# Chen001117/mappo

Hardware: AMD Instinct MI355X
Metric: agent-steps/sec (collect+GAE+PPO), MPE simple_spread 3-agent (higher is better)
Workload: dtype f32; 1 GPU; BASELINE configs[1]: MPE simple_spread shape, 3 agents, obs 18 / share_obs 54 / Discrete(5), n_rollout_threads=1024 in total (strong scaling: 1024 on rank 0 of 1), episode_length=25, MLP policy (mappo), ppo_epoch=10, num_mini_batch=1, lr 7e-4, env=synthetic; n_rollout_threads_global=1024, n_rollout_threads_rank0=1024, episode_length=25, num_agents=3, ppo_epoch=10, num_mini_batch=1, parallelism=dp1, rccl_ranks=0, exact_minibatch_order=False, hip_graph=True

## Files before the change

mappo_amd/csrc/insert_core.h:

```cpp
#pragma once
#include "common.h"

struct InsertArgs {
  const float *obs;  int64_t obs_sn, obs_sm;
  const float *rew;  int64_t rew_sn, rew_sm;
  const uint8_t *done; int64_t done_sn, done_sm;
  float *obs_dst, *share_dst, *rew_dst, *mask_dst;
  int N, M, D, centralized;
};

__device__ __forceinline__ void insert_mpe_body(const InsertArgs &p, int bid, int nb) {
  const int S = p.centralized ? p.M * p.D : p.D;
  const int64_t total = (int64_t)p.N * p.M * S;
  for (int64_t e = (int64_t)bid * blockDim.x + threadIdx.x; e < total; e += (int64_t)nb * blockDim.x) {
    const int64_t nm = e / S;
    const int j = (int)(e - nm * S);
    const int n = (int)(nm / p.M), m = (int)(nm - (int64_t)n * p.M);
    const int ms = p.centralized ? j / p.D : m, d = p.centralized ? j - ms * p.D : j;
    const float v = p.obs[n * p.obs_sn + ms * p.obs_sm + d];
    p.share_dst[e] = v;
    if (!p.centralized || ms == m) p.obs_dst[nm * p.D + d] = v;
    if (j == 0) {
      p.rew_dst[nm] = p.rew[n * p.rew_sn + m * p.rew_sm];
      p.mask_dst[nm] = p.done[n * p.done_sn + m * p.done_sm] ? 0.f : 1.f;
    }
  }
}

template <int U>
__device__ __forceinline__ void insert_mpe_episode_body(const InsertArgs &p, int64_t obs_st, int64_t rew_st, int64_t done_st, int T,
                                                        int bid, int nb) {
  const int S = p.centralized ? p.M * p.D : p.D;
  const int64_t R = (int64_t)p.N * p.M, RS = R * S, total = (int64_t)T * RS, nthr = (int64_t)nb * blockDim.x;
  for (int64_t e0 = (int64_t)bid * blockDim.x + threadIdx.x; e0 < total; e0 += U * nthr) {
    float v[U], rw[U];
    uint8_t dn[U];
    int64_t tn[U];
    int dd[U], jj[U];
#pragma unroll
    for (int u = 0; u < U; ++u) {
      const int64_t e = e0 + u * nthr;
      jj[u] = -1;
      if (e < total) {
        const int64_t t = e / RS, rem = e - t * RS, nm = rem / S;
        const int j = (int)(rem - nm * S);
        const int n = (int)(nm / p.M), m = (int)(nm - (int64_t)n * p.M);
        const int ms = p.centralized ? j / p.D : m, d = p.centralized ? j - ms * p.D : j;
        v[u] = p.obs[t * obs_st + n * p.obs_sn + ms * p.obs_sm + d];
        tn[u] = t * R + nm;
        dd[u] = (!p.centralized || ms == m) ? d : -1;
        jj[u] = j;
        if (j == 0) {
          rw[u] = p.rew[t * rew_st + n * p.rew_sn + m * p.rew_sm];
          dn[u] = p.done[t * done_st + n * p.done_sn + m * p.done_sm];
        }
      }
    }
    __builtin_amdgcn_sched_barrier(0);
    __builtin_amdgcn_s_waitcnt(0);
    __builtin_amdgcn_sched_barrier(0);
#pragma unroll
    for (int u = 0; u < U; ++u) {
      if (jj[u] < 0) continue;
      p.share_dst[e0 + u * nthr] = v[u];
      if (dd[u] >= 0) p.obs_dst[tn[u] * p.D + dd[u]] = v[u];
      if (jj[u] == 0) {
        p.rew_dst[tn[u]] = rw[u];
        p.mask_dst[tn[u]] = dn[u] != 0 ? 0.f : 1.f;
      }
    }
  }
}

struct SmacInsert {
  const float *obs, *share, *avail;
  const float *rew; int64_t rew_sn, rew_sm;
  const uint8_t *done; int64_t done_sn, done_sm;
  const uint8_t *bad;
  const float *h_a, *h_c;
  float *obs_dst, *share_dst, *avail_dst, *rew_dst, *mask_dst, *bad_dst, *active_dst, *ha_dst, *hc_dst;
  int N, M, D, S, A, H;
};
__device__ __forceinline__ bool env_done(const SmacInsert &p, int n) {
  bool all = true;
  for (int m = 0; m < p.M; ++m) all = all && p.done[n * p.done_sn + m * p.done_sm] != 0;
  return all;
}
__device__ __forceinline__ void insert_smac_body(const SmacInsert &p, int bid, int nb) {
  const int64_t tid = (int64_t)bid * blockDim.x + threadIdx.x, nthr = (int64_t)nb * blockDim.x;
  const int64_t R = (int64_t)p.N * p.M;
  for (int64_t e = tid; e < R * p.D; e += nthr) p.obs_dst[e] = p.obs[e];
  for (int64_t e = tid; e < R * p.S; e += nthr) p.share_dst[e] = p.share[e];
  if (p.avail)
    for (int64_t e = tid; e < R * p.A; e += nthr) p.avail_dst[e] = p.avail[e];
  for (int64_t e = tid; e < R; e += nthr) {
    const int n = (int)(e / p.M), m = (int)(e - (int64_t)n * p.M);
    const bool de = env_done(p, n), d = p.done[n * p.done_sn + m * p.done_sm] != 0;
    p.rew_dst[e] = p.rew[n * p.rew_sn + m * p.rew_sm];
    p.mask_dst[e] = de ? 0.f : 1.f;
    p.active_dst[e] = de ? 1.f : (d ? 0.f : 1.f);
    p.bad_dst[e] = (p.bad && p.bad[e]) ? 0.f : 1.f;
  }
  if (p.h_a) {
    const int h4 = p.H >> 2;
    for (int64_t e = tid; e < R * h4; e += nthr) {
      const int n = (int)((e / h4) / p.M);
      const float keep = env_done(p, n) ? 0.f : 1.f;
      float4 a = reinterpret_cast<const float4 *>(p.h_a)[e], c = reinterpret_cast<const float4 *>(p.h_c)[e];
      a.x *= keep; a.y *= keep; a.z *= keep; a.w *= keep;
      c.x *= keep; c.y *= keep; c.z *= keep; c.w *= keep;
      reinterpret_cast<float4 *>(p.ha_dst)[e] = a;
      reinterpret_cast<float4 *>(p.hc_dst)[e] = c;
    }
  }
}
```

mappo_amd/csrc/mlp_fwd16.h:

```cpp
#pragma once

#include "mlp_trunk16r.h"

template <bool RELU>
__device__ __forceinline__ void act_ln16(f32x4 (&acc)[4], const float *sG, const float *sBt, int q) {
  float s = 0.f;
#pragma unroll
  for (int b = 0; b < 4; ++b)
#pragma unroll
    for (int r = 0; r < 4; ++r) { acc[b][r] = act_fwd<RELU>(acc[b][r]); s += acc[b][r]; }
  const float mean = quad_sum16(s) * (1.f / HID);
  float v = 0.f;
#pragma unroll
  for (int b = 0; b < 4; ++b)
#pragma unroll
    for (int r = 0; r < 4; ++r) { const float c = acc[b][r] - mean; v += c * c; }
  const float rstd = 1.0f / sqrtf(quad_sum16(v) * (1.f / HID) + LN_EPS);
#pragma unroll
  for (int b = 0; b < 4; ++b) {
    const float4 g = *reinterpret_cast<const float4 *>(sG + 16 * b + 4 * q), t = *reinterpret_cast<const float4 *>(sBt + 16 * b + 4 * q);
    acc[b][0] = (acc[b][0] - mean) * rstd * g.x + t.x;
    acc[b][1] = (acc[b][1] - mean) * rstd * g.y + t.y;
    acc[b][2] = (acc[b][2] - mean) * rstd * g.z + t.z;
    acc[b][3] = (acc[b][3] - mean) * rstd * g.w + t.w;
// ... 126 lines not shown
  } else {
    f32x4 z[NBH > 0 ? NBH : 1];
#pragma unroll
    for (int bo = 0; bo < NBH; ++bo) {
      z[bo] = hd.bhv[bo];
      if (bo == 0 || A > 16) {
#pragma unroll
        for (int b = 0; b < 4; ++b)
#pragma unroll
          for (int r = 0; r < 4; ++r) z[bo] = mfma16(hd.wh[bo][b][r], h[b][r], z[bo]);
      }
    }
    if constexpr (DRAIN) { __builtin_amdgcn_sched_barrier(0); __builtin_amdgcn_s_waitcnt(0); __builtin_amdgcn_sched_barrier(0); }
    if constexpr (MODE == 0) {
      if (A == 1) { if (ok && q == 0) out[i] = z[0][0]; }
      else if (ok) {
#pragma unroll
        for (int r = 0; r < 4; ++r) { const int a = 4 * q + r; if (a < A) out[i * A + a] = z[0][r]; }
      }
    } else {
#pragma unroll
      for (int bo = 0; bo < NBH; ++bo)
#pragma unroll
        for (int r = 0; r < 4; ++r) { const int a = 16 * bo + 4 * q + r; if (a < A) tZ[j * TP + a] = z[bo][r]; }
      wave_lds_sync();
      if (ok && q == 0) {
        const uint64_t ctr = ctr_base + (ctr_dev ? *ctr_dev : 0ull);
        float action, lp;
        categorical_act_lane(tZ + j * TP, A, p.avail ? p.avail + i * A : nullptr, p.deterministic != 0, p.seed, ctr, (uint64_t)i, action, lp);
        actions[i] = action;
        logp[i] = lp;
      }
      wave_lds_sync();
    }
  }
}

template <bool RELU, int LN, int MODE>
__device__ __forceinline__ void forward16r_body(const FwdArgs &p, float *lds, const int bid, const int nb) {
  const int n_waves = blockDim.x / WAVE;
  const NetOff &o = p.off;
  const int lane = threadIdx.x & (WAVE - 1), wave = __builtin_amdgcn_readfirstlane((int)(threadIdx.x / WAVE)), j = lane & 15, q = lane >> 4;
  const int D = p.desc.in_dim, A = p.desc.out_dim;
  const int64_t n_tiles = (p.B + 15) / 16;
  float *tZ = lds + wave * 16 * TP;
  int64_t tile = (int64_t)bid * n_waves + wave;
  if (tile >= n_tiles) return;
  const float *P = p.params;
  auto load_x = [&](int64_t tl, f32x4 (&xv)[4]) {
    const int64_t i = tl * 16 + j;
    const int64_t row = i < p.B ? (p.rows ? (int64_t)p.rows[i] : i) : 0;
    const int64_t off = p.x_M ? (row / p.x_M) * p.x_sn + (row % p.x_M) * p.x_sm : row * D;
#pragma unroll
    for (int b = 0; b < 4; ++b)
#pragma unroll
      for (int r = 0; r < 4; ++r) xv[b][r] = p.x[off + min(16 * b + 4 * q + r, D - 1)];
  };
  f32x4 xn[4];
  load_x(tile, xn);
  Trunk16R<LN> tw;
  trunk16r_load<LN>(tw, P, o, p.desc, j, q);
  Head16R<MODE> hd;
  head16r_load<MODE>(hd, P, o, A, j, q);
  for (; tile < n_tiles; tile += (int64_t)nb * n_waves) {
    const int64_t i = tile * 16 + j;
    const bool ok = i < p.B;
    f32x4 x[4];
#pragma unroll
    for (int b = 0; b < 4; ++b) x[b] = xn[b];
    if (tile + (int64_t)nb * n_waves < n_tiles) load_x(tile + (int64_t)nb * n_waves, xn);
    tile16r_step<RELU, LN, MODE>(p, tw, hd, x, p.out, p.actions, p.logp, p.counter, p.counter_dev, tZ, i, ok, j, q);
  }
}

struct EpisodeSrc {
  const float *x0;
  int64_t x0_sn, x0_sm;
  const float *xp;
  int64_t xp_st, xp_sn, xp_sm;
};

template <bool RELU, int LN, int MODE>
__device__ __forceinline__ void episode16r_body(const FwdArgs &p, const EpisodeSrc &s, const int M, const int n_steps, const int n_last,
                                                float *last_out, float *lds, const int bid, const int nb) {
  const int n_waves = blockDim.x / WAVE;
  const int lane = threadIdx.x & (WAVE - 1), wave = __builtin_amdgcn_readfirstlane((int)(threadIdx.x / WAVE)), j = lane & 15, q = lane >> 4;
  const int D = p.desc.in_dim, A = p.desc.out_dim;
  const int64_t n_tiles = (p.B + 15) / 16;
  float *tZ = lds + wave * 16 * TP;
  const int64_t tile0 = (int64_t)bid * n_waves + wave, tstride = (int64_t)nb * n_waves;
  if (tile0 >= n_tiles) return;
  const int n_my = (int)((n_tiles - tile0 + tstride - 1) / tstride);
  const int n_items = n_steps * n_my;
  auto load_x = [&](int it, f32x4 (&xv)[4]) {
    const int t = it / n_my, k = it - t * n_my;
    const int64_t i = (tile0 + k * tstride) * 16 + j;
    const int64_t row = i < p.B ? i : 0;
    const float *base = t == 0 ? s.x0 : s.xp + (int64_t)(t - 1) * s.xp_st;
    const int64_t sn = t == 0 ? s.x0_sn : s.xp_sn, sm = t == 0 ? s.x0_sm : s.xp_sm;
    const int64_t off = (row / M) * sn + (row % M) * sm;
#pragma unroll
    for (int b = 0; b < 4; ++b)
#pragma unroll
      for (int r = 0; r < 4; ++r) xv[b][r] = base[off + min(16 * b + 4 * q + r, D - 1)];
  };
  f32x4 xn[4];
  load_x(0, xn);
  Trunk16R<LN> tw;
  trunk16r_load<LN>(tw, p.params, p.off, p.desc, j, q);
  Head16R<MODE> hd;
  head16r_load<MODE>(hd, p.params, p.off, A, j, q);
  const uint64_t ctr0 = p.counter + (MODE == 1 && p.counter_dev ? *p.counter_dev : 0ull);
  __builtin_amdgcn_sched_barrier(0);
  __builtin_amdgcn_s_waitcnt(0);
  __builtin_amdgcn_sched_barrier(0);
  for (int it = 0; it < n_items; ++it) {
    const int t = it / n_my, k = it - t * n_my;
    const int64_t i = (tile0 + k * tstride) * 16 + j;
    const bool ok = i < p.B;
    f32x4 x[4];
#pragma unroll
    for (int b = 0; b < 4; ++b) x[b] = xn[b];
    if (it + 1 < n_items) load_x(it + 1, xn);
    const int64_t so = (int64_t)t * p.B;
    float *out = MODE == 0 ? (t == n_last ? last_out : p.out + so) : nullptr;
    tile16r_step<RELU, LN, MODE, true>(p, tw, hd, x, out, MODE == 1 ? p.actions + so : nullptr, MODE == 1 ? p.logp + so : nullptr,
                                       ctr0 + (uint64_t)t, nullptr, tZ, i, ok, j, q);
  }
}

template <bool RELU, int LN, int MODE>
__device__ __forceinline__ void forward16_body(const FwdArgs &p, float *lds, const int bid, const int nb) {
  const int n_waves = blockDim.x / WAVE;
  const NetOff &o = p.off;
  const LdsMap &m = p.map;
  const int lane = threadIdx.x & (WAVE - 1), wave = __builtin_amdgcn_readfirstlane((int)(threadIdx.x / WAVE)), j = lane & 15, q = lane >> 4;
  const int D = p.desc.in_dim, Dp = (D + 1) & ~1, A = p.desc.out_dim;
  const int NG = (D + 3) >> 2;
  const int64_t n_tiles = (p.B + 15) / 16;
  const bool fnorm = p.desc.use_feature_norm != 0;
  const float inv_D = 1.0f / (float)D;
  float *tZ = lds + m.tiles + wave * m.wave_stride;
  bool staged = false;
  for (int64_t tile = (int64_t)bid * n_waves + wave; tile < n_tiles || !staged; tile += (int64_t)nb * n_waves) {
    const int64_t i = tile * 16 + j;
    const bool ok = tile < n_tiles && i < p.B;
    const int64_t row = ok ? (p.rows ? (int64_t)p.rows[i] : i) : 0;
    const int64_t off = p.x_M ? (row / p.x_M) * p.x_sn + (row % p.x_M) * p.x_sm : row * D;
    float xin[16];
#pragma unroll
    for (int g = 0; g < 16; ++g) xin[g] = p.x[off + min(4 * g + q, D - 1)];
    if (!staged) {
      stage_all_weights_1shot<LN>(lds, m, p.params, o, p.desc);
      __syncthreads();
      staged = true;
      if (tile >= n_tiles) break;
    }
#pragma unroll
    for (int g = 0; g < 16; ++g) xin[g] = (ok && 4 * g + q < D) ? xin[g] : 0.f;
    if (fnorm) {
      float s = 0.f;
#pragma unroll
      for (int g = 0; g < 16; ++g) s += xin[g];
      const float mean = quad_sum16(s) * inv_D;
      float v = 0.f;
#pragma unroll
      for (int g = 0; g < 16; ++g) { const float c = xin[g] - mean; v += c * c; }
      const int n_empty = 16 - max(0, min(16, (D - q + 3) >> 2));
      v -= (float)n_empty * mean * mean;
      const float rstd = 1.0f / sqrtf(fmaxf(quad_sum16(v), 0.f) * inv_D + LN_EPS);
#pragma unroll
      for (int g = 0; g < 16; ++g) xin[g] = (xin[g] - mean) * rstd * lds[m.fn_w + 4 * g + q] + lds[m.fn_b + 4 * g + q];
    }
    f32x4 h[4];
#pragma unroll
    for (int b = 0; b < 4; ++b) {
      const float4 bv = *reinterpret_cast<const float4 *>(lds + m.b1 + 16 * b + 4 * q);
      h[b][0] = bv.x; h[b][1] = bv.y; h[b][2] = bv.z; h[b][3] = bv.w;
    }
#pragma unroll
    for (int c = 0; c < 4; ++c) {
      if (4 * c < NG) {
#pragma unroll
        for (int gg = 0; gg < 4; ++gg) {
          const int g = 4 * c + gg;
          const float *rowp = lds + m.w1 + min(4 * g + q, Dp - 1) * WP + j;
#pragma unroll
          for (int b = 0; b < 4; ++b) h[b] = mfma16(rowp[16 * b], xin[g], h[b]);
        }
      }
    }
    forward16_tail<RELU, LN, MODE>(p, lds, m, h, i, ok, j, q, tZ);
  }
}
```

mappo_amd/csrc/mlp_impl.h:

```cpp
#include "mlp_core.h"
#include <stdlib.h>

#ifdef MLP_TU_MAIN
extern "C" int64_t mappo_net_param_count(const mappo_net_desc *desc) {
  if (!desc) return -1;
  return net_offsets(*desc).total;
}
#endif

struct LdsMap {
  int w1, w2[MAPPO_MAX_LAYER_N], wh;
  int fn_w, fn_b, b1, ln1_w, ln1_b, b2[MAPPO_MAX_LAYER_N], ln2_w[MAPPO_MAX_LAYER_N], ln2_b[MAPPO_MAX_LAYER_N], bh;
  int scratch;
  int tiles, x_rows, wave_stride, total;
  int fn_size;
};


__host__ __device__ inline LdsMap lds_map(const mappo_net_desc &d, int n_waves) {
  LdsMap m;
  int p = 0;
  const bool xw = d.in_dim > MAXD;
  const int Dp = xw ? MAXD : ((d.in_dim + 1) & ~1);
  m.fn_size = xw ? ((d.in_dim + 63) / 64) * 64 : MAXD;
// ... 522 lines not shown
    const int64_t base = tile * TS;
    int n_valid;
    TileStats<LN> st;
    if (!XWIDE) {
      n_valid = pf.n_valid;
      commit_rows(tX, tH + ((4 - ((m.x_rows * TP) & 3)) & 3), pf, D, magic, lane, p.desc.use_feature_norm != 0);
      wave_lds_sync();
      prefetch_rows(pf, p.x, p.rows, (tile + tile_stride) * TS, p.B, D, lane, p.x_sn, p.x_sm, p.x_M);
      tile_forward<RELU, LN>(lds, m, tX, tH, D, l31, half, st);
    } else {
      n_valid = (int)max((int64_t)0, min((int64_t)TS, p.B - base));
      const bool ok = l31 < n_valid;
      const int64_t row = ok ? (p.rows ? (int64_t)p.rows[base + l31] : base + l31) : 0;
      const float *xr = p.x + row * D;
      float mean0, rstd0;
      wide_row_stats(xr, D, ok, half, p.desc.use_feature_norm != 0, mean0, rstd0);
      tile_forward_wide<RELU, LN>(lds, m, p.params + o.w1, xr, ok, mean0, rstd0, tX, tH, D, l31, half, st);
    }
    if (MODE == 2) {
      const float *tL = tH + LN * HID * TP, *sG = lds + ln_w_of<LN>(m, LN), *sBt = lds + ln_b_of<LN>(m, LN);
      if (l31 < n_valid) {
#pragma unroll
        for (int t = 0; t < 2; ++t)
#pragma unroll
          for (int r = 0; r < 16; ++r) {
            const int f = 32 * t + ROWMAP(r, half);
            p.out[(int64_t)f * p.B + base + l31] = tL[f * TP + l31] * sG[f] + sBt[f];
          }
      }
      wave_lds_sync();
      continue;
    }
    const f32x16 z = head_forward(lds, m, tH + LN * HID * TP, lds + ln_w_of<LN>(m, LN), lds + ln_b_of<LN>(m, LN), l31, half);
    head_to_tile(tZ, z, A, l31, half);
    wave_lds_sync();
    if (MODE == 0) {
      for (int e = lane; e < n_valid * A; e += WAVE) {
        const int s = e / A, a = e - s * A;
        p.out[base * A + e] = tZ[s * TP + a];
      }
    } else {
      if (lane < n_valid) {
        const int64_t i = base + lane;
        const uint64_t ctr = p.counter + (p.counter_dev ? *p.counter_dev : 0ull);
        float action, logp;
        categorical_act_lane(tZ + lane * TP, A, p.avail ? p.avail + i * A : nullptr, p.deterministic != 0, p.seed, ctr, (uint64_t)i,
                             action, logp);
        p.actions[i] = action;
        p.logp[i] = logp;
      }
    }
    wave_lds_sync();
  }
}

template <bool RELU, int LN, int MODE, int XW>
__global__ __launch_bounds__(256, 1) void mlp_forward_kernel(FwdArgs p) {
  extern __shared__ __align__(16) float lds[];
  forward_body<RELU, LN, MODE, XW>(p, lds, blockIdx.x, gridDim.x);
}

#include "insert_core.h"
struct StepArgs {
  FwdArgs a, c;
  InsertArgs ins;
  int nA, nC, nI;
};
#include "mlp_fwd16.h"
template <bool RELU, int LN>
__global__ __launch_bounds__(256, 1) void rollout_step_kernel(StepArgs s) {
  extern __shared__ __align__(16) float lds[];
  const int bid = blockIdx.x;
  if (bid < s.nA) forward16r_body<RELU, LN, 1>(s.a, lds, bid, s.nA);
  else if (bid < s.nA + s.nC) forward16r_body<RELU, LN, 0>(s.c, lds, bid - s.nA, s.nC);
  else insert_mpe_body(s.ins, bid - s.nA - s.nC, s.nI);
}

struct EpisodeArgs {
  FwdArgs a, c;
  EpisodeSrc sa, sc;
  float *next_values;
  InsertArgs ins;
  int64_t ins_obs_st, ins_rew_st, ins_done_st;
  int T, M, nA, nC, nI;
};
template <bool RELU, int LN>
__global__ __launch_bounds__(256, 1) void rollout_episode_kernel(EpisodeArgs e) {
  extern __shared__ __align__(16) float lds[];
  const int bid = blockIdx.x;
  if (bid < e.nA) episode16r_body<RELU, LN, 1>(e.a, e.sa, e.M, e.T, -1, nullptr, lds, bid, e.nA);
  else if (bid < e.nA + e.nC) episode16r_body<RELU, LN, 0>(e.c, e.sc, e.M, e.T + 1, e.T, e.next_values, lds, bid - e.nA, e.nC);
  else insert_mpe_episode_body<8>(e.ins, e.ins_obs_st, e.ins_rew_st, e.ins_done_st, e.T, bid - e.nA - e.nC, e.nI);
}

template <bool RELU, int LN>
__global__ __launch_bounds__(256, 1) void features16_kernel(FwdArgs a) {
  extern __shared__ __align__(16) float lds[];
  forward16r_body<RELU, LN, 2>(a, lds, blockIdx.x, gridDim.x);
}
template <bool RELU, int LN>
__global__ __launch_bounds__(256, 1) void features16_dual_kernel(FwdArgs a, FwdArgs c, int nA) {
  extern __shared__ __align__(16) float lds[];
  if ((int)blockIdx.x < nA) forward16r_body<RELU, LN, 2>(a, lds, blockIdx.x, nA);
  else forward16r_body<RELU, LN, 2>(c, lds, blockIdx.x - nA, gridDim.x - nA);
}

#ifdef MLP_STAMPS
#define N_STAMPS 24
static unsigned long long *g_stamp_host = nullptr;
#define STAMP_DECL unsigned long long st_acc_[N_STAMPS] = {}; unsigned long long st_prev_ = __builtin_readcyclecounter();
#define STAMP(i)                                                          \
  do {                                                                    \
    __builtin_amdgcn_sched_barrier(0);                                    \
    const unsigned long long now_ = __builtin_readcyclecounter();         \
    st_acc_[i] += now_ - st_prev_;                                        \
    st_prev_ = now_;                                                      \
    __builtin_amdgcn_sched_barrier(0);                                    \
  } while (0)
#define STAMP_FLUSH()                                                                     \
  do {                                                                                    \
    if (p.stamps && threadIdx.x == 0)                                                     \
      for (int i_ = 0; i_ < N_STAMPS; ++i_) p.stamps[blockIdx.x * N_STAMPS + i_] = st_acc_[i_]; \
  } while (0)
#ifdef MLP_TU_MAIN
extern "C" int mappo_debug_set_stamps(unsigned long long *buf) { g_stamp_host = buf; return 0; }
#endif
#else
#define STAMP_DECL
#define STAMP(i) do { } while (0)
#define STAMP_FLUSH() do { } while (0)
#endif

struct UpdArgs {
  const float *params, *x;
  const int32_t *rows;
  float *slabs;
  int64_t slab_stride, slab_col0;
  mappo_net_desc desc;
  NetOff off;
  LdsMap map;
  int64_t B;
  int n_blocks;
  int n_regions;
  int p_red;
  int red_base;
  float *wide_ws;
  const float *dHT;
  int seq_nc;
  const float *dout;
  const float *avail, *actions, *old_logp, *adv, *active, *v_old, *returns, *vn_state;
  const double *mb_moments;
  double *partials;
  mappo_ppo_cfg cfg;
  unsigned long long *stamps;
};

__device__ __forceinline__ float tile_row_sum(const float *tile, int lane) {
  float s0 = 0.f, s1 = 0.f;
#pragma unroll 4
  for (int j = 0; j < TS; j += 2) { s0 += tile[lane * TP + j]; s1 += tile[lane * TP + j + 1]; }
  return s0 + s1;
}

__device__ __forceinline__ void regs_to_tile(float *tile, const f32x16 (&v)[2], int l31, int half) {
#pragma unroll
  for (int t = 0; t < 2; ++t)
#pragma unroll
    for (int r = 0; r < 16; ++r) tile[(32 * t + ROWMAP(r, half)) * TP + l31] = v[t][r];
}

template <bool RELU, bool AFFINE>
__device__ __forceinline__ void ln_act_backward(f32x16 (&dH)[2], float *tile, float mean, float rstd, uint32_t pos,
                                                const float *sG, float &gG, float &gB, int lane, int l31, int half) {
  f32x16 xh[2];
#pragma unroll
// ... 1067 lines not shown
    FwdArgs a = {}, c = {};
    a.params = actor_params; a.x = obs; a.avail = avail; a.actions = actions; a.logp = logp; a.desc = *actor_desc; a.B = B;
    a.deterministic = deterministic; a.seed = seed; a.counter = counter; a.counter_dev = counter_dev;
    a.off = net_offsets(a.desc); a.map = lds_map(a.desc, 8);
    c.params = critic_params; c.x = share_obs; c.out = values; c.desc = *critic_desc; c.B = B; c.off = net_offsets(c.desc); c.map = lds_map(c.desc, 8);
    Wide16Args wa, wc;
    size_t lba, lbc;
    dim3 ga, gc, ba, bc;
    bool sa, sc;
    if (int rcp = wide_forward_prepare(a, wa, lba, ga, ba, sa, "rollout_step")) return rcp;
    if (int rcp = wide_forward_prepare(c, wc, lbc, gc, bc, sc, "rollout_step")) return rcp;
    wa.x_M = M; wa.x_sn = obs_stride_n; wa.x_sm = obs_stride_m;
    wc.x_M = M; wc.x_sn = share_stride_n; wc.x_sm = share_stride_m;
    const int64_t n_groups = ((B + 15) / 16 + 7) / 8;
    const int nb = (int)(n_groups < NUM_CU / 2 ? n_groups : NUM_CU / 2);
    const int nA = actions ? nb : 0;
    const dim3 grid((unsigned)(nA + nb));
    const size_t lb = lba > lbc ? lba : lbc;
    if (full_step) {
      const size_t lw = sizeof(float) * ((size_t)HID * actor_desc->in_dim + HID);
      const size_t lf = lw > lb ? lw : lb;
      MAPPO_REQUIRE(lf <= 159 * 1024, "rollout_step: needs %zu B of LDS", lf);
      InsertArgs ins = {};
      if (fuse_ins) {
        wa.copy_dst = obs_dst; wc.copy_dst = share_dst;
        ins.rew = rewards; ins.rew_sn = rew_stride_n; ins.rew_sm = rew_stride_m; ins.done = dones; ins.done_sn = done_stride_n;
        ins.done_sm = done_stride_m; ins.rew_dst = rew_dst; ins.mask_dst = mask_dst; ins.N = (int)(B / M); ins.M = M;
      }
      const int rcf = actor_desc->use_relu
          ? wide16_launch_rollout_full_r<true>(actor_desc->layer_N, grid, lf, as_stream(stream), wa, a, wc, c, nA, fuse_ins ? &ins : nullptr)
          : wide16_launch_rollout_full_r<false>(actor_desc->layer_N, grid, lf, as_stream(stream), wa, a, wc, c, nA, fuse_ins ? &ins : nullptr);
      if (rcf) return rcf;
      MAPPO_CHECK_LAUNCH("rollout_step");
      return MAPPO_OK;
    }
    const int rcw = actor_desc->use_relu ? wide16_launch_rollout_step_r<true>(actor_desc->layer_N, grid, lb, as_stream(stream), wa, a, wc, c, nA)
                                         : wide16_launch_rollout_step_r<false>(actor_desc->layer_N, grid, lb, as_stream(stream), wa, a, wc, c, nA);
    if (rcw) return rcw;
    MAPPO_CHECK_LAUNCH("rollout_step");
    return MAPPO_OK;
  }
  const int64_t n_tiles = (B + 15) / 16;
  const int want = n_tiles >= 4 ? 4 : (n_tiles >= 2 ? 2 : 1);
  int nw = fit_waves(*actor_desc, want);
  const int nwc = fit_waves(*critic_desc, want);
  nw = nw < nwc ? nw : nwc;
  StepArgs s = {};
  s.a.params = actor_params; s.a.x = obs; s.a.avail = avail; s.a.actions = actions; s.a.logp = logp; s.a.desc = *actor_desc; s.a.B = B;
  s.a.deterministic = deterministic; s.a.seed = seed; s.a.counter = counter; s.a.counter_dev = counter_dev;
  s.a.x_sn = obs_stride_n; s.a.x_sm = obs_stride_m; s.a.x_M = M;
  s.a.off = net_offsets(s.a.desc); s.a.map = lds_map(s.a.desc, nw);
  s.c.params = critic_params; s.c.x = share_obs; s.c.out = values; s.c.desc = *critic_desc; s.c.B = B;
  s.c.x_sn = share_stride_n; s.c.x_sm = share_stride_m; s.c.x_M = M;
  s.c.off = net_offsets(s.c.desc); s.c.map = lds_map(s.c.desc, nw);
  const int totA = s.a.map.total, totC = s.c.map.total;
  const size_t lds_bytes = (size_t)(totA > totC ? totA : totC) * sizeof(float);
  MAPPO_REQUIRE(lds_bytes <= LDS_DYN_MAX, "rollout_step: needs %zu B of LDS", lds_bytes);
  int64_t nb = (n_tiles + nw - 1) / nw;
  if (nb > NUM_CU / 2) nb = NUM_CU / 2;
  s.nA = actions ? (int)nb : 0; s.nC = (int)nb; s.nI = 0;
  if (obs_dst) {
    InsertArgs &i = s.ins;
    i.obs = obs; i.obs_sn = obs_stride_n; i.obs_sm = obs_stride_m; i.rew = rewards; i.rew_sn = rew_stride_n; i.rew_sm = rew_stride_m;
    i.done = dones; i.done_sn = done_stride_n; i.done_sm = done_stride_m; i.obs_dst = obs_dst; i.share_dst = share_dst;
    i.rew_dst = rew_dst; i.mask_dst = mask_dst; i.N = (int)(B / M); i.M = M; i.D = actor_desc->in_dim; i.centralized = centralized;
    const int64_t total = B * (centralized ? (int64_t)M * i.D : i.D);
    int64_t ni = (total + 2047) / 2048;
    s.nI = (int)(ni > NUM_CU ? NUM_CU : ni);
  }
  dim3 grid((unsigned)(s.nA + s.nC + s.nI)), block(WAVE * nw);
  const bool relu = actor_desc->use_relu != 0;
  int rc;
  switch (actor_desc->layer_N) {
    case 0: rc = relu ? step_launch<true, 0>(grid, block, lds_bytes, as_stream(stream), s) : step_launch<false, 0>(grid, block, lds_bytes, as_stream(stream), s); break;
    case 1: rc = relu ? step_launch<true, 1>(grid, block, lds_bytes, as_stream(stream), s) : step_launch<false, 1>(grid, block, lds_bytes, as_stream(stream), s); break;
    default: rc = relu ? step_launch<true, 2>(grid, block, lds_bytes, as_stream(stream), s) : step_launch<false, 2>(grid, block, lds_bytes, as_stream(stream), s); break;
  }
  if (rc) return rc;
  MAPPO_CHECK_LAUNCH("rollout_step");
  return MAPPO_OK;
}

#define EPISODE_WAVES 1
template <bool R, int L>
static int episode_launch(dim3 grid, dim3 block, size_t lds_bytes, hipStream_t st, const EpisodeArgs &a) {
  hipLaunchKernelGGL((rollout_episode_kernel<R, L>), grid, block, lds_bytes, st, a);
  return MAPPO_OK;
}

extern "C" int mappo_rollout_episode(const float *actor_params, const mappo_net_desc *actor_desc, const float *critic_params,
                                     const mappo_net_desc *critic_desc, int32_t T, int32_t N, int32_t M, const float *env_obs,
                                     int64_t obs_stride_t, int64_t obs_stride_n, int64_t obs_stride_m, const float *rewards,
                                     int64_t rew_stride_t, int64_t rew_stride_n, int64_t rew_stride_m, const uint8_t *dones,
                                     int64_t done_stride_t, int64_t done_stride_n, int64_t done_stride_m, int32_t deterministic,
                                     uint64_t seed, uint64_t counter, const uint64_t *counter_dev, float *obs_buf, float *share_buf,
                                     float *rew_buf, float *mask_buf, float *actions, float *logp, float *values, float *next_values,
                                     int32_t centralized, mappo_stream_t stream) {
  if (int rc = check_desc(actor_desc, "rollout_episode")) return rc;
  if (int rc = check_desc(critic_desc, "rollout_episode")) return rc;
  MAPPO_REQUIRE(actor_desc->in_dim <= MAXD && critic_desc->in_dim <= MAXD, "rollout_episode: in_dim %d / %d: both networks must be narrow (<= %d)",
                actor_desc->in_dim, critic_desc->in_dim, MAXD);
  MAPPO_REQUIRE(actor_desc->layer_N == critic_desc->layer_N && actor_desc->use_relu == critic_desc->use_relu,
                "rollout_episode: actor and critic must share layer_N and the activation");
  MAPPO_REQUIRE(critic_desc->out_dim == 1, "rollout_episode: critic out_dim must be 1");
  MAPPO_REQUIRE(T >= 1 && N >= 1 && M >= 1, "rollout_episode: bad shape T=%d N=%d M=%d", T, N, M);
  MAPPO_REQUIRE(obs_stride_t >= 0 && obs_stride_n >= 0 && obs_stride_m >= 0 && rew_stride_t >= 0 && rew_stride_n >= 0 && rew_stride_m >= 0 &&
                done_stride_t >= 0 && done_stride_n >= 0 && done_stride_m >= 0, "rollout_episode: negative stride");
  const int D = actor_desc->in_dim;
  if (centralized)
    MAPPO_REQUIRE(critic_desc->in_dim == M * D && obs_stride_m == D, "rollout_episode: centralized critic needs in_dim M*D = %d (got %d) and "
                  "agent rows D apart in the env output (stride %lld)", M * D, critic_desc->in_dim, (long long)obs_stride_m);
  else
    MAPPO_REQUIRE(critic_desc->in_dim == D, "rollout_episode: critic in_dim %d != actor in_dim %d", critic_desc->in_dim, D);
  MAPPO_REQUIRE(actor_params && critic_params && env_obs && rewards && dones && obs_buf && share_buf && rew_buf && mask_buf && actions && logp &&
                values && next_values, "rollout_episode: bad arguments (null pointer)");
  MAPPO_CLEAR_STICKY();
  const int64_t B = (int64_t)N * M, S = critic_desc->in_dim;
  const int64_t n_tiles = (B + 15) / 16;
  int nw = EPISODE_WAVES;
  if (const char *ev = getenv("MAPPO_EPISODE_WAVES")) { const int v = atoi(ev); if (v == 1 || v == 2 || v == 4) nw = v; }
  int64_t nb = (n_tiles + nw - 1) / nw;
  if (nb > 2 * NUM_CU / nw) nb = 2 * NUM_CU / nw;
  EpisodeArgs e = {};
  e.a.params = actor_params; e.a.actions = actions; e.a.logp = logp; e.a.desc = *actor_desc; e.a.B = B; e.a.deterministic = deterministic;
  e.a.seed = seed; e.a.counter = counter; e.a.counter_dev = counter_dev; e.a.off = net_offsets(e.a.desc);
  e.c.params = critic_params; e.c.out = values; e.c.desc = *critic_desc; e.c.B = B; e.c.off = net_offsets(e.c.desc);
  e.sa = EpisodeSrc{obs_buf, (int64_t)M * D, D, env_obs, obs_stride_t, obs_stride_n, obs_stride_m};
  e.sc = EpisodeSrc{share_buf, (int64_t)M * S, S, env_obs, obs_stride_t, obs_stride_n, centralized ? 0 : obs_stride_m};
  e.next_values = next_values;
  InsertArgs &i = e.ins;
  i.obs = env_obs; i.obs_sn = obs_stride_n; i.obs_sm = obs_stride_m; i.rew = rewards; i.rew_sn = rew_stride_n; i.rew_sm = rew_stride_m;
  i.done = dones; i.done_sn = done_stride_n; i.done_sm = done_stride_m;
  i.obs_dst = obs_buf + B * D; i.share_dst = share_buf + B * S; i.rew_dst = rew_buf; i.mask_dst = mask_buf + B;
  i.N = N; i.M = M; i.D = D; i.centralized = centralized;
  e.ins_obs_st = obs_stride_t; e.ins_rew_st = rew_stride_t; e.ins_done_st = done_stride_t;
  e.T = T; e.M = M; e.nA = (int)nb; e.nC = (int)nb;
  int64_t n_ins_waves = ((int64_t)T * B * S + 64 * 8 * 2 - 1) / (64 * 8 * 2);
  const int64_t free_waves = 4 * NUM_CU - 2 * nb * nw;
  if (n_ins_waves > free_waves) n_ins_waves = free_waves < 64 ? 64 : free_waves;
  e.nI = (int)((n_ins_waves + nw - 1) / nw);
  const dim3 grid((unsigned)(e.nA + e.nC + e.nI)), block(WAVE * nw);
  const size_t lds_bytes = sizeof(float) * 16 * TP * nw;
  const bool relu = actor_desc->use_relu != 0;
  int rc;
  switch (actor_desc->layer_N) {
    case 0: rc = relu ? episode_launch<true, 0>(grid, block, lds_bytes, as_stream(stream), e) : episode_launch<false, 0>(grid, block, lds_bytes, as_stream(stream), e); break;
    case 1: rc = relu ? episode_launch<true, 1>(grid, block, lds_bytes, as_stream(stream), e) : episode_launch<false, 1>(grid, block, lds_bytes, as_stream(stream), e); break;
    default: rc = relu ? episode_launch<true, 2>(grid, block, lds_bytes, as_stream(stream), e) : episode_launch<false, 2>(grid, block, lds_bytes, as_stream(stream), e); break;
  }
  if (rc) return rc;
  MAPPO_CHECK_LAUNCH("rollout_episode");
  return MAPPO_OK;
}
#endif

#ifdef MLP_TU_MAIN
template <int MODE>
static int launch_forward(const FwdArgs &a_in, hipStream_t st, const char *who) {
  MAPPO_CLEAR_STICKY();
  const int64_t n_tiles = (a_in.B + TS - 1) / TS;
  const int LN = a_in.desc.layer_N;
  const int nw = fit_waves(a_in.desc, n_tiles >= 4 ? 4 : (n_tiles >= 2 ? 2 : 1));
  FwdArgs a = a_in;
  a.off = net_offsets(a.desc);
  a.map = lds_map(a.desc, nw);
  const size_t lds_bytes = (size_t)a.map.total * sizeof(float);
  MAPPO_REQUIRE(lds_bytes <= LDS_DYN_MAX, "%s: needs %zu B of LDS", who, lds_bytes);
  int64_t nb = (n_tiles + nw - 1) / nw;
  if (nb > NUM_CU) nb = NUM_CU;
  dim3 grid((unsigned)nb), block(WAVE * nw);
  {
    if (a.desc.in_dim > MAXD && a.desc.in_dim <= 512 && a.x_M == 0) {
      Wide16Args w;
      size_t lb;
      dim3 g2, b2;
      bool small;
      if (int rcp = wide_forward_prepare(a, w, lb, g2, b2, small, who)) return rcp;
      const int64_t nt16 = (a.B + 15) / 16;
      int64_t sk_max = WIDE_SK_MAX_TILES;
      if (const char *e = getenv("MAPPO_WIDE_SK_TILES")) sk_max = atoll(e);
      if (nt16 <= sk_max && !getenv("MAPPO_WIDE_NO_SK")) {
        const int64_t gsk = nt16 < NUM_CU ? nt16 : NUM_CU;
        if (int rcw = wide16_launch_forward_sk(MODE, a.desc.use_relu != 0, LN, dim3((unsigned)gsk), lb, st, w, a, who)) return rcw;
        MAPPO_CHECK_LAUNCH(who);
        return MAPPO_OK;
      }
      FwdArgs ar = a;
      ar.map = lds_map_tail(a.desc);
      const size_t lres = sizeof(float) * ((size_t)HID * 64 * ((a.desc.in_dim + 63) / 64) + HID + ar.map.tiles);
      if (MODE == 2 && LN <= 1 && nt16 >= 2 * 8 * NUM_CU && lres <= 159 * 1024 &&
          !(getenv("MAPPO_WIDE_RESIDENT") && atoi(getenv("MAPPO_WIDE_RESIDENT")) == 0)) {
        const int rcr = a.desc.use_relu ? wide16_launch_features_resident_r<true>(LN, g2, st, w, ar) : wide16_launch_features_resident_r<false>(LN, g2, st, w, ar);
        if (rcr) return rcr;
        MAPPO_CHECK_LAUNCH(who);
        return MAPPO_OK;
      }
      if (int rcw = wide16_launch_forward(MODE, a.desc.use_relu != 0, LN, small, g2, b2, lb, st, w, a, who)) return rcw;
      MAPPO_CHECK_LAUNCH(who);
      return MAPPO_OK;
    }
  }
#define FWD2(R, L, W)                                                                                          \
  do {                                                                                                         \
    static const hipError_t e_ = hipFuncSetAttribute((const void *)mlp_forward_kernel<R, L, MODE, W>,                      \
                                          hipFuncAttributeMaxDynamicSharedMemorySize, (int)LDS_DYN_MAX);       \
    if (e_ != hipSuccess) { mappo_set_error("%s: hipFuncSetAttribute: %s", who, hipGetErrorString(e_)); (void)hipGetLastError(); return MAPPO_ELAUNCH; } \
    PROF_LAUNCH(prof_id, (mlp_forward_kernel<R, L, MODE, W>), grid, block, lds_bytes, st, a);                   \
  } while (0)
#define FWD_W(R, L) do { if (xw == 2) FWD2(R, L, 2); else if (xw == 1) FWD2(R, L, 1); else FWD2(R, L, 0); } while (0)
  const bool relu = a.desc.use_relu != 0;
  const int xw = a.desc.in_dim > MAXD ? 2 : (a.desc.in_dim > 32 ? 1 : 0);
  const int prof_id = (MODE == 1) ? MAPPO_PROF_ACT : MAPPO_PROF_MLP_FWD;
  if (LN == 0) { if (relu) FWD_W(true, 0); else FWD_W(false, 0); }
  else if (LN == 1) { if (relu) FWD_W(true, 1); else FWD_W(false, 1); }
  else { if (relu) FWD_W(true, 2); else FWD_W(false, 2); }
#undef FWD_W
#undef FWD2
  MAPPO_CHECK_LAUNCH(who);
  return MAPPO_OK;
}

extern "C" int mappo_mlp_forward(const float *params, const mappo_net_desc *desc, const float *x, const int32_t *rows,
                                 int64_t B, float *out, mappo_stream_t stream) {
  if (int rc = check_desc(desc, "mlp_forward")) return rc;
// ... 620 lines not shown
```

Baseline: 72.23 million agent-steps/s.

## Rebalance rollout episode kernel waves with cost-model split and overlapped insert

The fused rollout-episode kernel now assigns work per wave instead of per block. Actor and critic waves stride over flattened (timestep, tile) items, and a small cost model picks the actor/critic wave split to balance their estimated load across 4*NUM_CU waves. By default no dedicated insert waves are allocated, so the env-insert copy runs on every wave after its network work finishes. The insert loop also uses 32-bit index math when the total fits and a deeper unroll of 16. The aim is to remove load imbalance and idle blocks between the three roles, at the cost of hard-coded cost constants and insert work now sitting on the same waves as the MLP work.

```diff
diff --git a/mappo_amd/csrc/insert_core.h b/mappo_amd/csrc/insert_core.h
--- a/mappo_amd/csrc/insert_core.h
+++ b/mappo_amd/csrc/insert_core.h
@@ -27,12 +27,12 @@
   }
 }
 
-template <int U>
-__device__ __forceinline__ void insert_mpe_episode_body(const InsertArgs &p, int64_t obs_st, int64_t rew_st, int64_t done_st, int T,
-                                                        int bid, int nb) {
+template <int U, typename I>
+__device__ __forceinline__ void insert_mpe_episode_run(const InsertArgs &p, int64_t obs_st, int64_t rew_st, int64_t done_st, int T,
+                                                       int w, int nw) {
   const int S = p.centralized ? p.M * p.D : p.D;
-  const int64_t R = (int64_t)p.N * p.M, RS = R * S, total = (int64_t)T * RS, nthr = (int64_t)nb * blockDim.x;
-  for (int64_t e0 = (int64_t)bid * blockDim.x + threadIdx.x; e0 < total; e0 += U * nthr) {
+  const int64_t R = (int64_t)p.N * p.M, RS = R * S, total = (int64_t)T * RS, nthr = (int64_t)nw * WAVE;
+  for (int64_t e0 = (int64_t)w * WAVE + (threadIdx.x & (WAVE - 1)); e0 < total; e0 += U * nthr) {
     float v[U], rw[U];
     uint8_t dn[U];
     int64_t tn[U];
@@ -42,17 +42,17 @@
       const int64_t e = e0 + u * nthr;
       jj[u] = -1;
       if (e < total) {
-        const int64_t t = e / RS, rem = e - t * RS, nm = rem / S;
-        const int j = (int)(rem - nm * S);
-        const int n = (int)(nm / p.M), m = (int)(nm - (int64_t)n * p.M);
+        const I t = (I)e / (I)RS, rem = (I)e - t * (I)RS, nm = rem / (I)S;
+        const int j = (int)(rem - nm * (I)S);
+        const int n = (int)(nm / (I)p.M), m = (int)(nm - (I)n * (I)p.M);
         const int ms = p.centralized ? j / p.D : m, d = p.centralized ? j - ms * p.D : j;
-        v[u] = p.obs[t * obs_st + n * p.obs_sn + ms * p.obs_sm + d];
-        tn[u] = t * R + nm;
+        v[u] = p.obs[(int64_t)t * obs_st + n * p.obs_sn + ms * p.obs_sm + d];
+        tn[u] = (int64_t)t * R + (int64_t)nm;
         dd[u] = (!p.centralized || ms == m) ? d : -1;
         jj[u] = j;
         if (j == 0) {
-          rw[u] = p.rew[t * rew_st + n * p.rew_sn + m * p.rew_sm];
-          dn[u] = p.done[t * done_st + n * p.done_sn + m * p.done_sm];
+          rw[u] = p.rew[(int64_t)t * rew_st + n * p.rew_sn + m * p.rew_sm];
+          dn[u] = p.done[(int64_t)t * done_st + n * p.done_sn + m * p.done_sm];
         }
       }
     }
@@ -70,6 +70,13 @@
       }
     }
   }
+}
+template <int U>
+__device__ __forceinline__ void insert_mpe_episode_body(const InsertArgs &p, int64_t obs_st, int64_t rew_st, int64_t done_st, int T,
+                                                        int w, int nw) {
+  const int64_t total = (int64_t)T * p.N * p.M * (p.centralized ? p.M * p.D : p.D);
+  if (total <= (int64_t)UINT32_MAX) insert_mpe_episode_run<U, uint32_t>(p, obs_st, rew_st, done_st, T, w, nw);
+  else insert_mpe_episode_run<U, int64_t>(p, obs_st, rew_st, done_st, T, w, nw);
 }
 
 struct SmacInsert {
diff --git a/mappo_amd/csrc/mlp_fwd16.h b/mappo_amd/csrc/mlp_fwd16.h
--- a/mappo_amd/csrc/mlp_fwd16.h
+++ b/mappo_amd/csrc/mlp_fwd16.h
@@ -232,19 +232,14 @@
 
 template <bool RELU, int LN, int MODE>
 __device__ __forceinline__ void episode16r_body(const FwdArgs &p, const EpisodeSrc &s, const int M, const int n_steps, const int n_last,
-                                                float *last_out, float *lds, const int bid, const int nb) {
-  const int n_waves = blockDim.x / WAVE;
-  const int lane = threadIdx.x & (WAVE - 1), wave = __builtin_amdgcn_readfirstlane((int)(threadIdx.x / WAVE)), j = lane & 15, q = lane >> 4;
+                                                float *last_out, float *tZ, const int w, const int nw) {
+  const int lane = threadIdx.x & (WAVE - 1), j = lane & 15, q = lane >> 4;
   const int D = p.desc.in_dim, A = p.desc.out_dim;
-  const int64_t n_tiles = (p.B + 15) / 16;
-  float *tZ = lds + wave * 16 * TP;
-  const int64_t tile0 = (int64_t)bid * n_waves + wave, tstride = (int64_t)nb * n_waves;
-  if (tile0 >= n_tiles) return;
-  const int n_my = (int)((n_tiles - tile0 + tstride - 1) / tstride);
-  const int n_items = n_steps * n_my;
-  auto load_x = [&](int it, f32x4 (&xv)[4]) {
-    const int t = it / n_my, k = it - t * n_my;
-    const int64_t i = (tile0 + k * tstride) * 16 + j;
+  const int64_t n_tiles = (p.B + 15) / 16, n_items = (int64_t)n_steps * n_tiles;
+  if (w >= n_items) return;
+  auto load_x = [&](int64_t it, f32x4 (&xv)[4]) {
+    const int t = (int)(it / n_tiles);
+    const int64_t i = (it - t * n_tiles) * 16 + j;
     const int64_t row = i < p.B ? i : 0;
     const float *base = t == 0 ? s.x0 : s.xp + (int64_t)(t - 1) * s.xp_st;
     const int64_t sn = t == 0 ? s.x0_sn : s.xp_sn, sm = t == 0 ? s.x0_sm : s.xp_sm;
@@ -255,7 +250,7 @@
       for (int r = 0; r < 4; ++r) xv[b][r] = base[off + min(16 * b + 4 * q + r, D - 1)];
   };
   f32x4 xn[4];
-  load_x(0, xn);
+  load_x(w, xn);
   Trunk16R<LN> tw;
   trunk16r_load<LN>(tw, p.params, p.off, p.desc, j, q);
   Head16R<MODE> hd;
@@ -264,14 +259,14 @@
   __builtin_amdgcn_sched_barrier(0);
   __builtin_amdgcn_s_waitcnt(0);
   __builtin_amdgcn_sched_barrier(0);
-  for (int it = 0; it < n_items; ++it) {
-    const int t = it / n_my, k = it - t * n_my;
-    const int64_t i = (tile0 + k * tstride) * 16 + j;
+  for (int64_t it = w; it < n_items; it += nw) {
+    const int t = (int)(it / n_tiles);
+    const int64_t i = (it - t * n_tiles) * 16 + j;
     const bool ok = i < p.B;
     f32x4 x[4];
 #pragma unroll
     for (int b = 0; b < 4; ++b) x[b] = xn[b];
-    if (it + 1 < n_items) load_x(it + 1, xn);
+    if (it + nw < n_items) load_x(it + nw, xn);
     const int64_t so = (int64_t)t * p.B;
     float *out = MODE == 0 ? (t == n_last ? last_out : p.out + so) : nullptr;
     tile16r_step<RELU, LN, MODE, true>(p, tw, hd, x, out, MODE == 1 ? p.actions + so : nullptr, MODE == 1 ? p.logp + so : nullptr,
diff --git a/mappo_amd/csrc/mlp_impl.h b/mappo_amd/csrc/mlp_impl.h
--- a/mappo_amd/csrc/mlp_impl.h
+++ b/mappo_amd/csrc/mlp_impl.h
@@ -628,15 +628,17 @@
   float *next_values;
   InsertArgs ins;
   int64_t ins_obs_st, ins_rew_st, ins_done_st;
-  int T, M, nA, nC, nI;
+  int T, M, wA, wC, wI0, wAll;
 };
 template <bool RELU, int LN>
 __global__ __launch_bounds__(256, 1) void rollout_episode_kernel(EpisodeArgs e) {
   extern __shared__ __align__(16) float lds[];
-  const int bid = blockIdx.x;
-  if (bid < e.nA) episode16r_body<RELU, LN, 1>(e.a, e.sa, e.M, e.T, -1, nullptr, lds, bid, e.nA);
-  else if (bid < e.nA + e.nC) episode16r_body<RELU, LN, 0>(e.c, e.sc, e.M, e.T + 1, e.T, e.next_values, lds, bid - e.nA, e.nC);
-  else insert_mpe_episode_body<8>(e.ins, e.ins_obs_st, e.ins_rew_st, e.ins_done_st, e.T, bid - e.nA - e.nC, e.nI);
+  const int wave = __builtin_amdgcn_readfirstlane((int)(threadIdx.x / WAVE));
+  const int gw = (int)blockIdx.x * (int)(blockDim.x / WAVE) + wave;
+  float *tZ = lds + wave * 16 * TP;
+  if (gw < e.wA) episode16r_body<RELU, LN, 1>(e.a, e.sa, e.M, e.T, -1, nullptr, tZ, gw, e.wA);
+  else if (gw < e.wA + e.wC) episode16r_body<RELU, LN, 0>(e.c, e.sc, e.M, e.T + 1, e.T, e.next_values, tZ, gw - e.wA, e.wC);
+  if (gw >= e.wI0 && gw < e.wAll) insert_mpe_episode_body<16>(e.ins, e.ins_obs_st, e.ins_rew_st, e.ins_done_st, e.T, gw - e.wI0, e.wAll - e.wI0);
 }
 
 template <bool RELU, int LN>
@@ -1870,6 +1872,14 @@
 }
 
 #define EPISODE_WAVES 1
+#define EPISODE_COST_A 150
+#define EPISODE_COST_C 134
+static int env_int(const char *name, int dflt, int lo, int hi) {
+  const char *ev = getenv(name);
+  if (!ev) return dflt;
+  const int v = atoi(ev);
+  return v < lo ? lo : (v > hi ? hi : v);
+}
 template <bool R, int L>
 static int episode_launch(dim3 grid, dim3 block, size_t lds_bytes, hipStream_t st, const EpisodeArgs &a) {
   hipLaunchKernelGGL((rollout_episode_kernel<R, L>), grid, block, lds_bytes, st, a);
@@ -1905,10 +1915,20 @@
   MAPPO_CLEAR_STICKY();
   const int64_t B = (int64_t)N * M, S = critic_desc->in_dim;
   const int64_t n_tiles = (B + 15) / 16;
-  int nw = EPISODE_WAVES;
-  if (const char *ev = getenv("MAPPO_EPISODE_WAVES")) { const int v = atoi(ev); if (v == 1 || v == 2 || v == 4) nw = v; }
-  int64_t nb = (n_tiles + nw - 1) / nw;
-  if (nb > 2 * NUM_CU / nw) nb = 2 * NUM_CU / nw;
+  int nw = env_int("MAPPO_EPISODE_WAVES", EPISODE_WAVES, 1, 4);
+  if (nw != 1 && nw != 2) nw = 4;
+  const int n_ins = env_int("MAPPO_EPISODE_INS_WAVES", 0, 0, 4 * NUM_CU - 2);
+  const int n_net = env_int("MAPPO_EPISODE_NET_WAVES", 4 * NUM_CU - n_ins, 2, 4 * NUM_CU);
+  const int64_t cost_a = env_int("MAPPO_EPISODE_COST_A", EPISODE_COST_A, 1, 1000), cost_c = EPISODE_COST_C;
+  const int64_t items_a = (int64_t)T * n_tiles, items_c = (int64_t)(T + 1) * n_tiles;
+  int64_t wa = 1, best = -1;
+  for (int64_t a = 1; a < n_net; ++a) {
+    const int64_t la = (items_a + a - 1) / a * cost_a, lc = (items_c + (n_net - a) - 1) / (n_net - a) * cost_c;
+    const int64_t l = la > lc ? la : lc;
+    if (best < 0 || l < best) { best = l; wa = a; }
+  }
+  const int64_t wc = n_net - wa > items_c ? items_c : n_net - wa;
+  if (wa > items_a) wa = items_a;
   EpisodeArgs e = {};
   e.a.params = actor_params; e.a.actions = actions; e.a.logp = logp; e.a.desc = *actor_desc; e.a.B = B; e.a.deterministic = deterministic;
   e.a.seed = seed; e.a.counter = counter; e.a.counter_dev = counter_dev; e.a.off = net_offsets(e.a.desc);
@@ -1922,12 +1942,10 @@
   i.obs_dst = obs_buf + B * D; i.share_dst = share_buf + B * S; i.rew_dst = rew_buf; i.mask_dst = mask_buf + B;
   i.N = N; i.M = M; i.D = D; i.centralized = centralized;
   e.ins_obs_st = obs_stride_t; e.ins_rew_st = rew_stride_t; e.ins_done_st = done_stride_t;
-  e.T = T; e.M = M; e.nA = (int)nb; e.nC = (int)nb;
-  int64_t n_ins_waves = ((int64_t)T * B * S + 64 * 8 * 2 - 1) / (64 * 8 * 2);
-  const int64_t free_waves = 4 * NUM_CU - 2 * nb * nw;
-  if (n_ins_waves > free_waves) n_ins_waves = free_waves < 64 ? 64 : free_waves;
-  e.nI = (int)((n_ins_waves + nw - 1) / nw);
-  const dim3 grid((unsigned)(e.nA + e.nC + e.nI)), block(WAVE * nw);
+  e.T = T; e.M = M; e.wA = (int)wa; e.wC = (int)wc;
+  e.wI0 = n_ins > 0 ? e.wA + e.wC : 0;
+  e.wAll = e.wA + e.wC + n_ins;
+  const dim3 grid((unsigned)((e.wAll + nw - 1) / nw)), block(WAVE * nw);
   const size_t lds_bytes = sizeof(float) * 16 * TP * nw;
   const bool relu = actor_desc->use_relu != 0;
   int rc;
```

Result: faster. 75.35 million agent-steps/s (median of 6 runs) (+4.3%).
